# applied-ai-lab/genesis

Measured on AMD Instinct MI355X. Metric: training images/sec (fwd+bwd+GECO step), GENESIS-V2 K=7 64x64, higher is better.
Workload: dtype f32

## Files before the change

### genesis_amd/csrc/gx_norm.hip

```cpp
#include "gx_common.h"

#include <vector>

namespace {

struct View {
    float* ptr;
    int ctot;
    int c0;
    int mode;
    const float* proj;
    int projC;
    const float* pgate;
    int nsplit;
    size_t sstride;
};

struct InSrc {
    const float* p;
    int nsplit;
    size_t stride;
    const float* bias;
    float* ysum;
};
// ... 454 lines not shown
            store_view4(d0, n, c, r, col, H, W, o);
            if (d1.ptr) store_view4(d1, n, c, r, col, H, W, o);
            am = fmaxf(fmaxf(am, fmaxf(o[0], o[1])), fmaxf(o[2], o[3]));
        }
    }
    if (amax_parts) {
#pragma unroll
        for (int of = 32; of >= 1; of >>= 1) am = fmaxf(am, __shfl_xor(am, of, 64));
        if (lane == 0) amr[wave] = am;
        __syncthreads();
        if (threadIdx.x == 0) {
            float r = 0.f;
            for (int i = 0; i < (int)(blockDim.x >> 6); ++i) r = fmaxf(r, amr[i]);
            amax_parts[blockIdx.x] = r;
        }
    }
}

__device__ __forceinline__ f32x4 staged_grad(const float* gsl, const float (&pw)[8], int ctot, int HW, int i4) {
    f32x4 g = {0.f, 0.f, 0.f, 0.f};
#pragma unroll
    for (int q = 0; q < 8; ++q)
        if (q < ctot) g += pw[q] * reinterpret_cast<const f32x4*>(gsl)[q * (HW >> 2) + i4];
    return g;
}

template <int F, int UPW, bool STAGE>
__global__ void __launch_bounds__(1024)
gn_relu_bwd_reg_kernel(const float* __restrict__ y, const float* __restrict__ gamma, const float* __restrict__ beta,
                       const float* __restrict__ mean_in, const float* __restrict__ rstd_in,
// ... 485 lines not shown
    if (HW >= 256 || (W % 4) != 0 || cpg > 64 || m > 4096) return 0;
    return gx_round_up(m / 4, 64);
}

inline float* gn_take_link_out(const float* tensor, int ctot, int c0, int mode, int C, unsigned nwg, size_t covered, bool second_copy = false) {
    GxAmaxLink& L = gx_amax_link();
    const bool link_ok = !second_copy && L.parts && !L.tensor && tensor && c0 == 0 && mode == 0 && ctot == C && covered == L.numel;
    return gx_amax_producer_out(tensor, link_ok, nwg, covered);
}
template <int F, int UPW>
void launch_fwd_reg(dim3 grid, dim3 block, hipStream_t s, const InSrc src, const float* gamma, const float* beta, int C, int H,
                    int W, int groups, int P, float eps, View d0, View d1, float* mean, float* rstd) {
    float* ap = d0.ptr ? gn_take_link_out(d0.ptr, d0.ctot, d0.c0, d0.mode, C, grid.x, (size_t)(grid.x / groups) * C * H * W, d1.ptr != nullptr) : nullptr;
    hipLaunchKernelGGL((gn_relu_fwd_reg_kernel<F, UPW>), grid, block, 0, s, src, gamma, beta, C, H, W, groups, P, eps, d0, d1,
                       mean, rstd, ap);
}
template <int F, int UPW>
bool launch_bwd_stage(dim3 grid, dim3 block, hipStream_t s, size_t lds, const float* y, const float* gamma,
                      const float* beta, const float* mean, const float* rstd, int C, int H, int W, int groups, int P,
                      View g0, View g1, float* dy, float* part, float* wpart, float* bpart) {
    if (UPW != 1 || block.x != 1024 || g0.ctot != 4) return false;
    float* amax_parts = gn_take_link_out(dy, C, 0, 0, C, grid.x, (size_t)(grid.x / groups) * C * H * W);
    constexpr bool KEEP = F < 8;
    static bool attr_set = false;
    if (!attr_set) {
        (void)hipFuncSetAttribute(reinterpret_cast<const void*>(&gn_relu_bwd_stage_kernel<F, 4, true, KEEP>),
                                  hipFuncAttributeMaxDynamicSharedMemorySize, 150 * 1024);
        (void)hipFuncSetAttribute(reinterpret_cast<const void*>(&gn_relu_bwd_stage_kernel<F, 4, false, KEEP>),
                                  hipFuncAttributeMaxDynamicSharedMemorySize, 150 * 1024);
        attr_set = true;
// ... 374 lines not shown
                               beta, C, H, W, groups, pl.P, eps, d0, d1, mean, rstd);
        else if (st)
            hipLaunchKernelGGL(gn_relu_fwd_small_kernel, dim3(N * groups), dim3(st), 0, (hipStream_t)stream, src, gamma,
                               beta, C, H, W, groups, eps, d0, d1, mean, rstd);
        else {
            float* ap = dst0 ? gn_take_link_out(dst0, d0.ctot, d0.c0, d0.mode, C, (unsigned)(N * groups), (size_t)N * C * H * W, dst1 != nullptr) : nullptr;
            if (vec)
                hipLaunchKernelGGL(gn_relu_fwd_kernel<true>, dim3(N * groups), dim3(threads), 0, (hipStream_t)stream, src,
                                   gamma, beta, C, H, W, groups, eps, d0, d1, mean, rstd, ap);
            else
                hipLaunchKernelGGL(gn_relu_fwd_kernel<false>, dim3(N * groups), dim3(threads), 0, (hipStream_t)stream, src,
                                   gamma, beta, C, H, W, groups, eps, d0, d1, mean, rstd, ap);
        }
    }
    GX_CHECK_LAUNCH("gx_gn_relu_fwd");
    return GX_OK;
}

size_t gx_gn_relu_bwd_ws_bytes(int N, int C) { return (size_t)N * C * 3 * sizeof(float); }
size_t gx_gn_relu_bwd_proj_ws_bytes(int N, int C, int H, int W, int groups, int Cout) {
    size_t b = gx_gn_relu_bwd_ws_bytes(N, C);
    if (proj_split_ok(C, H, W, groups, Cout))
        b += ((size_t)N * groups * (H * W / kSplitPix) * kSplitRec + (size_t)N * groups * 2) * sizeof(float);
    return b;
}

static int gn_relu_bwd_impl(const float* y, const float* gamma, const float* beta, const float* mean,
                            const float* rstd, int N, int C, int H, int W, int groups, const View& v0, const View& v1,
                            float* dy, float* dgamma, float* dbeta, float* dbias, void* ws, size_t ws_bytes,
                            gx_stream_t stream, float* wpart = nullptr, float* bpart = nullptr);
// ... 140 lines not shown
```

### genesis_amd/csrc/gx_slots.hip

```cpp
#include "gx_common.h"

#include <cstdlib>

namespace {

constexpr int KMAX = 16;

__device__ __forceinline__ float block_sum_f(float v, float* red) {
    v = gx_wave_sum(v);
    const int lane = threadIdx.x & 63, wave = threadIdx.x >> 6, nw = blockDim.x >> 6;
    __syncthreads();
    if (lane == 0) red[wave] = v;
    __syncthreads();
    float s = 0.f;
    for (int i = 0; i < nw; ++i) s += red[i];
    return s;
}
__device__ __forceinline__ double block_sum_dd(double v, double* red) {
    v = gx_wave_sum_d(v);
    const int lane = threadIdx.x & 63, wave = threadIdx.x >> 6, nw = blockDim.x >> 6;
    __syncthreads();
    if (lane == 0) red[wave] = v;
    __syncthreads();
    double s = 0.0;
// ... 126 lines not shown
#pragma unroll
        for (int k = 0; k < KMAX; ++k) {
            if (k < K) {
                const float g = gsh[k * C + c];
                a[k] += g * fv;
                d += m[k] * g;
            }
        }
        dfb[(size_t)c * HW] = d;
    }
#pragma unroll
    for (int k = 0; k < KMAX; ++k)
        if (k < K) dlog_m[k * kstride + (size_t)b * HW + p] = m[k] * (a[k] + gmsum[(size_t)b * K + k]);
}

template <int KT>
__global__ void __launch_bounds__(256)
maskpool_bwd_vec_kernel(const float* __restrict__ f, const float* __restrict__ log_m, const float* __restrict__ gS,
                        const float* __restrict__ gmsum, int B, int C, int HW, int Krt, float* __restrict__ df,
                        float* __restrict__ dlog_m) {
    const int K = KT ? KT : Krt;
    constexpr int KMAX = KT ? KT : ::KMAX;
    extern __shared__ __attribute__((aligned(16))) float sm[];
    float* gsh = sm;
    f32x4* ared = reinterpret_cast<f32x4*>(sm + ((K * C + 3) & ~3));
    const int lane = threadIdx.x & 63, wave = threadIdx.x >> 6;
    const int b = blockIdx.x;
    const int p = (blockIdx.y * 64 + lane) * 4;
    for (int i = threadIdx.x; i < K * C; i += blockDim.x) gsh[i] = gS[(size_t)b * K * C + i];
    __syncthreads();
    const bool act = p < HW;
    const size_t kstride = (size_t)B * HW;
    f32x4 m[KMAX], a[KMAX];
#pragma unroll
    for (int k = 0; k < KMAX; ++k) {
        a[k][0] = 0.f; a[k][1] = 0.f; a[k][2] = 0.f; a[k][3] = 0.f;
        m[k] = a[k];
        if (k < K && act) {
            const f32x4 lm = *reinterpret_cast<const f32x4*>(log_m + k * kstride + (size_t)b * HW + p);
#pragma unroll
            for (int e = 0; e < 4; ++e) m[k][e] = expf(lm[e]);
        }
    }
    const int cper = (C + 3) / 4;
    const int cbeg = wave * cper, cend = (cbeg + cper < C) ? cbeg + cper : C;
    if (act) {
        const float* fb = f + (size_t)b * C * HW + p;
        float* dfb = df + (size_t)b * C * HW + p;
#pragma unroll 4
        for (int c = cbeg; c < cend; ++c) {
            const f32x4 fv = *reinterpret_cast<const f32x4*>(fb + (size_t)c * HW);
            f32x4 d = {0.f, 0.f, 0.f, 0.f};
#pragma unroll
            for (int k = 0; k < KMAX; ++k) {
                if (k < K) {
                    const float g = gsh[k * C + c];
                    a[k] += g * fv;
                    d += m[k] * g;
                }
            }
            *reinterpret_cast<f32x4*>(dfb + (size_t)c * HW) = d;
        }
    }
#pragma unroll
    for (int k = 0; k < KMAX; ++k)
        if (k < K) ared[(wave * K + k) * 64 + lane] = a[k];
    __syncthreads();
    if (wave == 0 && act) {
#pragma unroll
        for (int k = 0; k < KMAX; ++k) {
            if (k < K) {
                const f32x4 t = (ared[(0 * K + k) * 64 + lane] + ared[(1 * K + k) * 64 + lane]) +
                                (ared[(2 * K + k) * 64 + lane] + ared[(3 * K + k) * 64 + lane]);
                *reinterpret_cast<f32x4*>(dlog_m + k * kstride + (size_t)b * HW + p) =
                    m[k] * (t + gmsum[(size_t)b * K + k]);
            }
        }
    }
}

constexpr float LOG_SQRT_2PI = 0.91893853320467274178f;

template <bool BWD, int KT>
__global__ void __launch_bounds__(256)
mixture_kernel(const float* __restrict__ x, const float* __restrict__ dec, int B, int HW, int Krt, float std_,
               int pixel_bound, float* __restrict__ recon, float* __restrict__ x_r, float* __restrict__ log_m_r,
               float* __restrict__ err_part, const float* __restrict__ g_err, float* __restrict__ ddec,
               const float* __restrict__ log_w, float* __restrict__ dlog_w, float std_first, int DC) {
    const int K = KT ? KT : Krt;
    constexpr int KMAX = KT ? KT : ::KMAX;
// ... 450 lines not shown
#undef GX_MP_FWD
    }
    GX_CHECK_LAUNCH("gx_maskpool_fwd");
    return GX_OK;
}

int gx_maskpool_bwd(const float* f, const float* log_m, const float* gS, const float* gmsum, int B, int C, int H,
                    int W, int K, float* df, float* dlog_m, gx_stream_t stream) {
    GX_CHECK_ARG(f && log_m && gS && gmsum && df && dlog_m, "gx_maskpool_bwd: null pointer");
    GX_CHECK_ARG(B > 0 && C > 0 && K >= 1 && K <= KMAX && H > 0 && W > 0, "gx_maskpool_bwd: bad dims (K<=16)");
    const int HW = H * W;
    {
        GxProf pf(KID_MASKPOOL_BWD, (hipStream_t)stream, 4.0 * B * K * C * HW, 4.0 * B * HW * (2.0 * C + 2.0 * K));
        if (gx_vec4_ok(HW, f, log_m, df, dlog_m)) {
#define GX_MP_BWD(KT_)                                                                                                 \
            hipLaunchKernelGGL(maskpool_bwd_vec_kernel<KT_>, dim3(B, gx_ceil_div(HW, 256)), dim3(256),                \
                               (size_t)(((K * C + 3) & ~3) + 4 * K * 64 * 4) * sizeof(float), (hipStream_t)stream, f,   \
                               log_m, gS, gmsum, B, C, HW, K, df, dlog_m)
            if (K == 7) GX_MP_BWD(7); else if (K == 5) GX_MP_BWD(5); else if (K == 11) GX_MP_BWD(11); else GX_MP_BWD(0);
#undef GX_MP_BWD
        }
        else
            hipLaunchKernelGGL(maskpool_bwd_kernel, dim3(B, gx_ceil_div(HW, 256)), dim3(256),
                               (size_t)K * C * sizeof(float), (hipStream_t)stream, f, log_m, gS, gmsum, B, C, HW, K, df,
                               dlog_m);
    }
    GX_CHECK_LAUNCH("gx_maskpool_bwd");
    return GX_OK;
}

size_t gx_mixture_ws_bytes(int B, int H, int W) { return (size_t)B * gx_ceil_div(H * W, 256) * sizeof(float); }

static int mixture_fwd_impl(const float* x, const float* dec, const float* log_w, int dec_ch, int B, int H, int W, int K,
                            float std_first, float pixel_std, int pixel_bound, float* recon, float* x_r,
                            float* log_m_r, float* err, void* ws, size_t ws_bytes, gx_stream_t stream) {
    GX_CHECK_ARG(x && dec && recon && x_r && err && ws, "gx_mixture_fwd: null pointer");
    GX_CHECK_ARG(B > 0 && K >= 1 && K <= KMAX && pixel_std > 0.f, "gx_mixture_fwd: bad dims (K<=16)");
    GX_CHECK_ARG(ws_bytes >= gx_mixture_ws_bytes(B, H, W), "gx_mixture_fwd: workspace too small");
    const int HW = H * W, nb = gx_ceil_div(HW, 256);
    hipStream_t s = (hipStream_t)stream;
    {
        GxProf pf(KID_MIXTURE_FWD, s, 0.0, 4.0 * B * HW * (6.0 + 8.0 * K));
// ... 297 lines not shown
```

### genesis_amd/functions.py

```python
import os

import torch
import torch.nn.functional as F

from . import _lib
from . import autostep as _auto
from . import hip_ops as hip
from . import precision as _precision

GROUPS = 8
EPS = 1e-5

class _StepState(object):
    __slots__ = ('direct_param_grads', 'direct_written', 'async_wgrad', 'side_stream', 'keep_alive', 'early_flush')

    def __init__(self):
        self.direct_param_grads = False
        self.direct_written = set()
        self.async_wgrad = False
        self.side_stream = None
        self.keep_alive = []
        self.early_flush = None


# ... 385 lines not shown
    @staticmethod
    def forward(ctx, enc_feat, seg_w, seg_gamma, seg_beta, conv_w, conv_b, gate, uv, log_sigma, rand_pixel, K, kernel,
                seed_idx, min_mass, feat_w, feat_gamma, feat_beta):
        x = enc_feat.contiguous()
        ctx.am_x = getattr(enc_feat, '_gx_amax', None)
        ctx.params = (seg_w, seg_gamma, seg_beta, conv_w, conv_b, gate, log_sigma, feat_w, feat_gamma, feat_beta)
        w2 = conv_w.detach().view(conv_w.shape[0], -1)
        y, yf, ctx.pair_ws = hip.conv3x3_pair_fwd(x, seg_w, feat_w, amax_in=ctx.am_x)
        mean, rstd = hip.gn_relu_fwd(y, seg_gamma, seg_beta, GROUPS, EPS, None)
        colour = hip.conv1x1_gn_fwd(y, mean, rstd, seg_gamma, seg_beta, GROUPS, w2, conv_b, gate, uv)
        ctx.ls_dtype = log_sigma.dtype
        ls64 = log_sigma.detach().to(torch.float64)
        res = hip.icsbp_fwd(colour, ls64, rand_pixel.contiguous(), K, kernel, seed_idx, min_mass)
        log_m, log_s, seeds, idx = res[:4]
        ctx.nsteps = res[4] if min_mass > 0.0 else None
        f = torch.empty_like(yf)
        meanf, rstdf = hip.gn_relu_fwd(yf, feat_gamma, feat_beta, GROUPS, EPS, (f, 0, 0))
        ctx.save_for_backward(x, y, mean, rstd, ls64, colour, seeds, idx, yf, meanf, rstdf)
        ctx.kernel = kernel
        ctx.mark_non_differentiable(idx)
        ctx.set_materialize_grads(False)
        if ctx.nsteps is not None:
            ctx.mark_non_differentiable(ctx.nsteps)
            return log_m, log_s, colour, seeds, idx, ctx.nsteps, f
        return log_m, log_s, colour, seeds, idx, f

    @staticmethod
    def backward(ctx, g_log_m, *rest):
        _refuse_grads('SegFeatHeadsFn', rest)
        x, y, mean, rstd, ls64, colour, seeds, idx, yf, meanf, rstdf = ctx.saved_tensors
        seg_w, seg_gamma, seg_beta, conv_w, conv_b, gate, log_sigma, feat_w, feat_gamma, feat_beta = ctx.params
        g_f = rest[-1]
        if g_log_m is None:
            g_log_m = colour.new_zeros(seeds.shape[0] + 1, colour.shape[0], 1, colour.shape[2], colour.shape[3])
        if g_f is None:
            g_f = torch.zeros_like(yf)
        ols = _gout(log_sigma) if ctx.ls_dtype == torch.float64 and log_sigma.dim() == 0 else None
        dcolour, dls = hip.icsbp_bwd(colour, ls64, seeds, idx, g_log_m.contiguous(), ctx.kernel, out_dls=ols,
                                     nsteps=ctx.nsteps)
        w2 = conv_w.detach().view(conv_w.shape[0], -1)
        ow, ob, og = _gout(conv_w), _gout(conv_b), (_gout(gate) if gate is not None else None)
        osw, osg, osb = _gout(seg_w), _gout(seg_gamma), _gout(seg_beta)
        fused = hip.conv1x1_gn_bwd_fused(y, seg_gamma, seg_beta, mean, rstd, GROUPS, dcolour, w2, conv_b, gate, False,
                                         out_gn=(osg, osb, None), out_conv=(ow, ob, og))
        if fused is not None:
            dy, (dgamma, dbeta, _), (dw, db, dgate) = fused
        else:
            dw, db, dgate = hip.conv1x1_gn_wgrad(y, mean, rstd, seg_gamma, seg_beta, GROUPS, dcolour, w2, conv_b, gate,
                                                 out=(ow, ob, og))
            dy, dgamma, dbeta, _ = hip.gn_relu_bwd_proj(y, seg_gamma, seg_beta, mean, rstd, GROUPS, dcolour, w2, False,
                                                        out=(osg, osb, None), gate=gate)
        am_s = (hip.take_amax(), ctx.am_x)
        dsw = _wgrad(lambda: hip.conv3x3_wgrad(x, dy, out=osw, amax=am_s), osw, x, dy)
        ofw, ofg, ofb = _gout(feat_w), _gout(feat_gamma), _gout(feat_beta)
        dyf, dfgamma, dfbeta, _ = hip.gn_relu_bwd(yf, feat_gamma, feat_beta, meanf, rstdf, GROUPS, (g_f.contiguous(), 0, 0),
                                                  out=(ofg, ofb, None))
        am_f = (hip.take_amax(), ctx.am_x)
        dfw = _wgrad(lambda: hip.conv3x3_wgrad(x, dyf, out=ofw, amax=am_f), ofw, x, dyf)
        dx = hip.conv3x3_pair_dgrad(dy, dyf, seg_w, feat_w, ctx.pair_ws, amax_in=[am_s[0], am_f[0]]) if ctx.needs_input_grad[0] else None
        return (dx, _ret(osw, dsw), _ret(osg, dgamma), _ret(osb, dbeta), _ret(ow, dw.view(conv_w.shape)), _ret(ob, db),
                _ret(og, dgate), None, _ret(ols, dls.to(ctx.ls_dtype)), None, None, None, None, None,
                _ret(ofw, dfw), _ret(ofg, dfgamma), _ret(ofb, dfbeta))


@ctx_bound
class MaskPoolFn(torch.autograd.Function):
    @staticmethod
    def forward(ctx, f, log_m):
        f = f.contiguous()
        log_m = log_m.contiguous()
        S, msum = hip.maskpool_fwd(f, log_m)
        ctx.save_for_backward(f, log_m)
        return S, msum

    @staticmethod
    def backward(ctx, gS, gmsum):
        f, log_m = ctx.saved_tensors
# ... 933 lines not shown
```

### genesis_amd/genesisv2_config.py

```python
import math

import numpy as np
import torch
import torch.nn as nn
import torch.nn.functional as F
from torch.distributions.normal import Normal

from genesis_amd import autostep
from genesis_amd import compat as _compat

_compat.install()

from attrdict import AttrDict
from forge import flags

from genesis_amd import functions as fn
from genesis_amd.lazy import Lazy, LazyAttrDict, SlotList
from genesis_amd import hip_ops as hip

flags.DEFINE_integer('feat_dim', 64, 'Number of features and latents.')
flags.DEFINE_string('kernel', 'gaussian', '{laplacian, gaussian, epanechnikov')
flags.DEFINE_boolean('semiconv', True, 'Use semi-convolutional embeddings.')
flags.DEFINE_boolean('dynamic_K', False, 'Dynamic K.')
flags.DEFINE_boolean('klm_loss', False, 'KL mask regulariser.')
# ... 209 lines not shown
        K, D = self.K_steps, self.feat_dim
        dev = x.device
        uv, _ = self._grid(dev)
        enc_feat = fn.UNetEncoderFn.apply(x, self.encoder.num_blocks, 8, *self.encoder.flat_params())
        if rand_pixel is None and eps is None and getattr(self, 'noise', None) is not None:
            rand_pixel, eps = self.noise((B, 1, H, W), (K, B, D), dev)
        if rand_pixel is None:
            rand_pixel = torch.rand(B, 1, H, W, device=dev)
        ap = self.att_process
        if ap.semiconv:
            cw, cb, gate, addend = ap.colour_head.conv.weight, ap.colour_head.conv.bias, ap.colour_head.gate.gate, uv
        else:
            cw, cb, gate, addend = ap.colour_head.weight, ap.colour_head.bias, None, None
        seg_params = self.seg_head.params()
        min_mass = 20.0 if self.dynamic_K else 0.0
        f = None
        if fn.heads_pairable(enc_feat, seg_params[0], cw, self.feat_head[0].params()[0]):
            res = fn.SegFeatHeadsFn.apply(enc_feat, *seg_params, cw, cb, gate, addend, ap.log_sigma, rand_pixel, K,
                                          ap.kernel, seed_idx, min_mass, *self.feat_head[0].params())
            res, f = res[:-1], res[-1]
        elif fn.seg_head_fusable(enc_feat, seg_params[0], cw):
            res = fn.SegICSBPFn.apply(enc_feat, *seg_params, cw, cb, gate, addend, ap.log_sigma, rand_pixel, K, ap.kernel,
                                      seed_idx, min_mass)
        else:
            seg = fn.ConvGNReLUFn.apply(enc_feat, *seg_params)
            res = fn.ICSBPFn.apply(seg, cw, cb, gate, addend, ap.log_sigma, rand_pixel, K, ap.kernel, seed_idx, min_mass)
        log_m, log_s, colour, seeds, idx = res[:5]
        dyn_batched = False
        if self.dynamic_K:
            if B == 1:
                n = int(res[5][0])
                K = n + 1
                log_m, log_s = log_m[:K], log_s[:K]
                seeds, idx = seeds[:min(n + 1, self.K_steps - 1)], idx[:min(n + 1, self.K_steps - 1)]
                if eps is not None:
                    eps = eps[:K]
            else:
                dyn_batched = True
        if f is None:
            f = fn.ConvGNReLUFn.apply(enc_feat, *self.feat_head[0].params())
        S, msum = fn.MaskPoolFn.apply(f, log_m)
        ln = self.z_head[0]
        zh = fn.PooledHeadFn.apply(fn.linear(S, self.feat_head[1].weight), msum, self.feat_head[1].bias,
                                   ln.weight, ln.bias, ln.eps)
        if eps is None:
            eps = torch.randn(K, B, D, device=dev)
        zh = fn.linear(zh, self.z_head[1].weight, self.z_head[1].bias, 'relu')
        zh = fn.linear(zh, self.z_head[3].weight, self.z_head[3].bias)
        z, mu, sigma, log_q = fn.PosteriorFn.apply(zh, eps)
        err, recon, x_r, log_m_r = self._decode(z, x, self.klm_loss and not self.detach_mr_in_klm)
        kl = self._component_kl(z, log_q)
        t = dict(err=err, kl=kl, recon=recon, log_m=log_m, log_s=log_s, x_r=x_r, log_m_r=log_m_r, colour=colour, seeds=seeds,
                 idx=idx, mu=mu, sigma=sigma, z=z)
        if self.klm_loss:
            t['kl_m'] = fn.CategoricalKLFn.apply(log_m, log_m_r.detach() if self.detach_mr_in_klm else log_m_r)
        t['dyn_batched'] = dyn_batched
# ... 75 lines not shown
```

### genesis_amd/hip_ops.py

```python
import ctypes
import os

import torch

from . import _lib
from ._lib import GenesisHipError

F32 = torch.float32
KERNELS = {'gaussian': 0, 'laplacian': 1, 'epanechnikov': 2}


def _chk(t, name, dtype=F32):
    if t is None:
        return
    if not t.is_cuda:
        raise GenesisHipError('%s: the HIP hot path needs device tensors (got %s); there is no CPU fallback'
                              % (name, t.device))
    if t.dtype != dtype:
        raise GenesisHipError('%s: expected %s, got %s' % (name, dtype, t.dtype))
    if not t.is_contiguous():
        raise GenesisHipError('%s: tensor must be contiguous' % name)


def _p(t):
# ... 542 lines not shown
    msum = torch.empty(B, K, dtype=F32, device=f.device)
    _lib.call('gx_maskpool_fwd', _p(f), _p(log_m), B, C, H, W, K, _p(S), _p(msum), _stream())
    return S, msum


def maskpool_bwd(f, log_m, gS, gmsum):
    _chk(gS, 'maskpool_bwd.gS'); _chk(gmsum, 'maskpool_bwd.gmsum')
    B, C, H, W = f.shape
    K = log_m.shape[0]
    df = torch.empty_like(f)
    dlog_m = torch.empty_like(log_m)
    _lib.call('gx_maskpool_bwd', _p(f), _p(log_m), _p(gS), _p(gmsum), B, C, H, W, K, _p(df), _p(dlog_m), _stream())
    return df, dlog_m


def mixture_fwd(x, dec, K, pixel_std, pixel_bound=True):
    _chk(x, 'mixture.x'); _chk(dec, 'mixture.dec')
    B, _, H, W = x.shape
    assert dec.shape == (K * B, 4, H, W), dec.shape
    dev = x.device
    recon = torch.empty(B, 3, H, W, dtype=F32, device=dev)
    x_r = torch.empty(K, B, 3, H, W, dtype=F32, device=dev)
    log_m_r = torch.empty(K, B, 1, H, W, dtype=F32, device=dev)
    err = torch.empty(B, dtype=F32, device=dev)
    nb = _lib.query('gx_mixture_ws_bytes', B, H, W)
    ws = _ws(nb, dev)
    _lib.call('gx_mixture_fwd', _p(x), _p(dec), B, H, W, K, float(pixel_std), int(bool(pixel_bound)), _p(recon),
              _p(x_r), _p(log_m_r), _p(err), _p(ws), nb, _stream())
    return err, recon, x_r, log_m_r

# ... 867 lines not shown
```

### include/genesis_hip.h

```cpp
#ifndef GENESIS_HIP_H
#define GENESIS_HIP_H
#include <stddef.h>
#include <stdint.h>

#ifdef __cplusplus
extern "C" {
#endif

typedef void* gx_stream_t;

#define GX_OK 0
#define GX_EINVAL (-1)
#define GX_ELAUNCH (-2)
#define GX_EDATA (-3)

const char* gx_last_error(void);
int gx_version(void);

size_t gx_conv3x3_ws_bytes(int N, int Cin, int Cout, int H, int W);
int gx_conv3x3_fwd(const float* x, const float* w, float* y, int N, int Cin, int Cout, int H, int W,
                   void* ws, size_t ws_bytes, gx_stream_t stream);
int gx_conv3x3_dgrad(const float* dy, const float* w, float* dx, int N, int Cin, int Cout, int H, int W,
                     void* ws, size_t ws_bytes, gx_stream_t stream);
int gx_conv3x3_dgrad_parts(const float* dy, const float* w, float* dx, int N, int Cin, int Cout, int H, int W, void* ws,
// ... 40 lines not shown
int gx_deconv5x5s2_fwd(const float* x, const float* w, const float* bias, float* y, int N, int Cin, int Cout,
                       int Hin, int Win, void* ws, size_t ws_bytes, gx_stream_t stream);
size_t gx_deconv5x5s2_gn_stats_ws_bytes(int N, int Cin, int Cout, int Hin, int Win);
int gx_deconv5x5s2_gn_stats_fwd(const float* x, const float* w, const float* bias, float* y, int N, int Cin, int Cout,
                                int Hin, int Win, int groups, float eps, float* mean, float* rstd, int* fused,
                                void* ws, size_t ws_bytes, gx_stream_t stream);
int gx_deconv5x5s2_dgrad(const float* dy, const float* w, float* dx, int N, int Cin, int Cin_out, int Cout,
                         int Hin, int Win, void* ws, size_t ws_bytes, gx_stream_t stream);
size_t gx_deconv5x5s2_wgrad_ws_bytes(int N, int Cin, int Cout, int Hin, int Win);
int gx_deconv5x5s2_wgrad(const float* x, const float* dy, float* dw, int N, int Cin, int Cout, int Hin, int Win,
                         void* ws, size_t ws_bytes, gx_stream_t stream);

int gx_gn_relu_fwd(const float* y, const float* gamma, const float* beta, int N, int C, int H, int W, int groups,
                   float eps, float* dst0, int dst0_ctot, int dst0_c0, int dst0_mode, float* dst1, int dst1_ctot,
                   int dst1_c0, int dst1_mode, float* mean, float* rstd, gx_stream_t stream);
size_t gx_gn_relu_bwd_ws_bytes(int N, int C);
int gx_gn_relu_bwd(const float* y, const float* gamma, const float* beta, const float* mean, const float* rstd,
                   int N, int C, int H, int W, int groups, const float* g0, int g0_ctot, int g0_c0, int g0_mode,
                   const float* g1, int g1_ctot, int g1_c0, int g1_mode, float* dy, float* dgamma, float* dbeta,
                   float* dbias, void* ws, size_t ws_bytes, gx_stream_t stream);
int gx_gn_relu_bwd_parts(const float* y, const float* gamma, const float* beta, const float* mean, const float* rstd,
                         int N, int C, int H, int W, int groups, const float* g0, int g0_ctot, int g0_c0, int g0_mode,
                         int g0_nsplit, size_t g0_split_stride, const float* g1, int g1_ctot, int g1_c0, int g1_mode,
                         int g1_nsplit, size_t g1_split_stride, float* dy, float* dgamma, float* dbeta, float* dbias, void* ws,
                         size_t ws_bytes, gx_stream_t stream);
int gx_gn_relu_bwd_proj(const float* y, const float* gamma, const float* beta, const float* mean, const float* rstd,
                        int N, int C, int H, int W, int groups, const float* g_out, int Cout, const float* w,
                        const float* gate, float* dy, float* dgamma, float* dbeta, float* dbias, float* wpart,
                        float* bpart, void* ws, size_t ws_bytes, gx_stream_t stream);
int gx_gn_relu_bwd_proj_fuses_wgrad(int C, int H, int W, int groups, int Cout);
// ... 7 lines not shown
size_t gx_icsbp_bwd_ws_bytes(int B, int H, int W, int K);
int gx_icsbp_bwd(const float* colour, const double* log_sigma, const float* seeds, const int64_t* seed_idx,
                 const float* g_log_m, int B, int C, int H, int W, int K, int kernel_type, float* dcolour,
                 double* dlog_sigma, void* ws, size_t ws_bytes, gx_stream_t stream);
int gx_icsbp_fwd_dyn(const float* colour, const double* log_sigma, const float* rand_pixel, const int64_t* seed_idx_in,
                     int B, int C, int H, int W, int K, int kernel_type, float min_mass, float* log_m, float* log_s,
                     float* seeds, int64_t* seed_idx_out, int* nsteps, gx_stream_t stream);
int gx_icsbp_bwd_dyn(const float* colour, const double* log_sigma, const float* seeds, const int64_t* seed_idx,
                     const float* g_log_m, const int* nsteps, int B, int C, int H, int W, int K, int kernel_type,
                     float* dcolour, double* dlog_sigma, void* ws, size_t ws_bytes, gx_stream_t stream);

int gx_maskpool_fwd(const float* f, const float* log_m, int B, int C, int H, int W, int K, float* S, float* msum,
                    gx_stream_t stream);
int gx_maskpool_bwd(const float* f, const float* log_m, const float* gS, const float* gmsum, int B, int C, int H,
                    int W, int K, float* df, float* dlog_m, gx_stream_t stream);

size_t gx_mixture_ws_bytes(int B, int H, int W);
int gx_mixture_fwd(const float* x, const float* dec, int B, int H, int W, int K, float pixel_std, int pixel_bound,
                   float* recon, float* x_r, float* log_m_r, float* err, void* ws, size_t ws_bytes,
                   gx_stream_t stream);
int gx_mixture_bwd(const float* x, const float* dec, const float* g_err, int B, int H, int W, int K,
                   float pixel_std, int pixel_bound, float* ddec, gx_stream_t stream);

int gx_conv1x1_fwd(const float* x, const float* w, const float* bias, const float* gate, const float* addend,
                   int N, int Cin, int Cout, int H, int W, float* y, gx_stream_t stream);
size_t gx_conv1x1_bwd_ws_bytes(int N, int Cin, int Cout, int H, int W);
int gx_conv1x1_bwd(const float* x, const float* dy, const float* w, const float* bias, const float* gate, int N,
                   int Cin, int Cout, int H, int W, float* dx, float* dw, float* db, float* dgate, void* ws,
                   size_t ws_bytes, gx_stream_t stream);
int gx_conv1x1_bwd_ex(const float* x, const float* dy, const float* w, const float* bias, const float* gate, int N,
// ... 315 lines not shown
```

Baseline: 11730.

## Fuse feature GroupNorm+ReLU with mask pooling and recompute features in pool backward

```diff
diff --git a/genesis_amd/csrc/gx_norm.hip b/genesis_amd/csrc/gx_norm.hip
--- a/genesis_amd/csrc/gx_norm.hip
+++ b/genesis_amd/csrc/gx_norm.hip
@@ -492,6 +492,114 @@
             for (int i = 0; i < (int)(blockDim.x >> 6); ++i) r = fmaxf(r, amr[i]);
             amax_parts[blockIdx.x] = r;
         }
+    }
+}
+
+constexpr int kPoolKMax = 16;
+constexpr size_t kPoolLdsBudget = 128 * 1024;
+template <int F, int UPW>
+__global__ void __launch_bounds__(1024)
+gn_relu_fwd_pool_kernel(const float* __restrict__ x, const float* __restrict__ gamma, const float* __restrict__ beta,
+                        const float* __restrict__ log_m, int C, int H, int W, int groups, int P, int K, float eps,
+                        float* __restrict__ mean_out, float* __restrict__ rstd_out, float* __restrict__ S,
+                        float* __restrict__ msum) {
+    __shared__ double red[16 * 2 + 2];
+    __shared__ double upool[32][kPoolKMax];
+    extern __shared__ __attribute__((aligned(16))) float msl[];
+    const int n = blockIdx.x / groups, gidx = blockIdx.x % groups;
+    const int N = gridDim.x / groups;
+    const int cpg = C / groups, HW = H * W;
+    const int m = cpg * HW;
+    const int lane = threadIdx.x & 63, wave = threadIdx.x >> 6;
+    const int q4 = (HW >> 2) / P;
+    const size_t slab_off = ((size_t)n * C + (size_t)gidx * cpg) * HW;
+    f32x4 xr[UPW][F];
+    double acc[2] = {0.0, 0.0};
+#pragma unroll
+    for (int u = 0; u < UPW; ++u) {
+        const int unit = wave * UPW + u;
+        const int cl = unit / P, part = unit - cl * P;
+#pragma unroll
+        for (int j = 0; j < F; ++j)
+            xr[u][j] = *reinterpret_cast<const f32x4*>(x + slab_off + (size_t)cl * HW + 4 * (size_t)(part * q4 + j * 64 + lane));
+    }
+    {
+        const int HW4 = HW >> 2, lHW4 = __ffs(HW4) - 1;
+#pragma unroll 2
+        for (int i = threadIdx.x; i < K * HW4; i += blockDim.x) {
+            const int k = i >> lHW4, p4 = i & (HW4 - 1);
+            const f32x4 lm = *reinterpret_cast<const f32x4*>(log_m + ((size_t)k * N + n) * HW + 4 * (size_t)p4);
+            f32x4 mv;
+#pragma unroll
+            for (int e = 0; e < 4; ++e) mv[e] = expf(lm[e]);
+            reinterpret_cast<f32x4*>(msl)[i] = mv;
+        }
+    }
+#pragma unroll
+    for (int u = 0; u < UPW; ++u)
+#pragma unroll
+        for (int j = 0; j < F; ++j) {
+            const f32x4 v = xr[u][j];
+            acc[0] += ((double)v[0] + (double)v[1]) + ((double)v[2] + (double)v[3]);
+            acc[1] += ((double)v[0] * v[0] + (double)v[1] * v[1]) + ((double)v[2] * v[2] + (double)v[3] * v[3]);
+        }
+    block_sum_multi<2>(acc, red);
+    const double mean = acc[0] / m;
+    double var = acc[1] / m - mean * mean;
+    if (var < 0.0) var = 0.0;
+    const float meanf = (float)mean;
+    const float rstdf = (float)(1.0 / sqrt(var + (double)eps));
+    if (threadIdx.x == 0) { mean_out[blockIdx.x] = meanf; rstd_out[blockIdx.x] = rstdf; }
+#pragma unroll
+    for (int u = 0; u < UPW; ++u) {
+        const int unit = wave * UPW + u;
+        const int cl = unit / P;
+        const int c = gidx * cpg + cl;
+        const float gm = gamma[c], bt = beta[c];
+#pragma unroll
+        for (int j = 0; j < F; ++j)
+#pragma unroll
+            for (int e = 0; e < 4; ++e) {
+                const float t = (xr[u][j][e] - meanf) * rstdf * gm + bt;
+                xr[u][j][e] = t > 0.f ? t : 0.f;
+            }
+    }
+    const f32x4* ms4 = reinterpret_cast<const f32x4*>(msl);
+    for (int k = 0; k < K; ++k) {
+#pragma unroll
+        for (int u = 0; u < UPW; ++u) {
+            const int unit = wave * UPW + u;
+            const int cl = unit / P, part = unit - cl * P;
+            double s0 = 0.0, s1 = 0.0, s2 = 0.0, s3 = 0.0;
+#pragma unroll
+            for (int j = 0; j < F; ++j) {
+                const f32x4 mv = ms4[k * (HW >> 2) + part * q4 + j * 64 + lane];
+                s0 += (double)(mv[0] * xr[u][j][0]);
+                s1 += (double)(mv[1] * xr[u][j][1]);
+                s2 += (double)(mv[2] * xr[u][j][2]);
+                s3 += (double)(mv[3] * xr[u][j][3]);
+            }
+            const double s = gx_wave_sum_d((s0 + s1) + (s2 + s3));
+            if (lane == 0) upool[unit][k] = s;
+        }
+    }
+    if (gidx == 0) {
+        for (int k = wave; k < K; k += (int)(blockDim.x >> 6)) {
+            double s0 = 0.0, s1 = 0.0, s2 = 0.0, s3 = 0.0;
+            for (int i = lane; i < (HW >> 2); i += 64) {
+                const f32x4 mv = ms4[k * (HW >> 2) + i];
+                s0 += (double)mv[0]; s1 += (double)mv[1]; s2 += (double)mv[2]; s3 += (double)mv[3];
+            }
+            const double s = gx_wave_sum_d((s0 + s1) + (s2 + s3));
+            if (lane == 0) msum[(size_t)n * K + k] = (float)s;
+        }
+    }
+    __syncthreads();
+    for (int t = threadIdx.x; t < cpg * K; t += blockDim.x) {
+        const int cl = t / K, k = t - cl * K;
+        double s = 0.0;
+        for (int p = 0; p < P; ++p) s += upool[cl * P + p][k];
+        S[((size_t)n * K + k) * C + gidx * cpg + cl] = (float)s;
     }
 }
 
@@ -1007,6 +1115,19 @@
     float* ap = d0.ptr ? gn_take_link_out(d0.ptr, d0.ctot, d0.c0, d0.mode, C, grid.x, (size_t)(grid.x / groups) * C * H * W, d1.ptr != nullptr) : nullptr;
     hipLaunchKernelGGL((gn_relu_fwd_reg_kernel<F, UPW>), grid, block, 0, s, src, gamma, beta, C, H, W, groups, P, eps, d0, d1,
                        mean, rstd, ap);
+}
+template <int F, int UPW>
+void launch_fwd_pool(dim3 grid, dim3 block, hipStream_t s, size_t lds, const float* y, const float* gamma, const float* beta,
+                     const float* log_m, int C, int H, int W, int groups, int P, int K, float eps, float* mean, float* rstd,
+                     float* S, float* msum) {
+    static bool attr_set = false;
+    if (!attr_set) {
+        (void)hipFuncSetAttribute(reinterpret_cast<const void*>(&gn_relu_fwd_pool_kernel<F, UPW>),
+                                  hipFuncAttributeMaxDynamicSharedMemorySize, (int)kPoolLdsBudget);
+        attr_set = true;
+    }
+    hipLaunchKernelGGL((gn_relu_fwd_pool_kernel<F, UPW>), grid, block, lds, s, y, gamma, beta, log_m, C, H, W, groups, P, K, eps,
+                       mean, rstd, S, msum);
 }
 template <int F, int UPW>
 bool launch_bwd_stage(dim3 grid, dim3 block, hipStream_t s, size_t lds, const float* y, const float* gamma,
@@ -1411,6 +1532,37 @@
         }
     }
     GX_CHECK_LAUNCH("gx_gn_relu_fwd");
+    return GX_OK;
+}
+
+int gx_gn_relu_pool_covers(const float* y, const float* log_m, size_t lm_stride_k, size_t lm_stride_n, size_t lm_stride_h,
+                           size_t lm_stride_w, int N, int C, int H, int W, int groups, int K) {
+    if (N <= 0 || C <= 0 || groups <= 0 || C % groups || K < 1 || K > kPoolKMax) return 0;
+    if (H < 2 || W < 2 || !gx_is_pow2(H) || !gx_is_pow2(W)) return 0;
+    if (!plan_reg(C / groups, H, W).ok) return 0;
+    if ((size_t)K * H * W * sizeof(float) > kPoolLdsBudget) return 0;
+    if (gx_maskpool_bwd_norm_lds_bytes(C, K) > 64 * 1024) return 0;
+    if (lm_stride_w != 1 || lm_stride_h != (size_t)W || lm_stride_n != (size_t)H * W || lm_stride_k != (size_t)N * H * W) return 0;
+    if (((reinterpret_cast<uintptr_t>(y) | reinterpret_cast<uintptr_t>(log_m)) & 15) != 0) return 0;
+    return 1;
+}
+
+int gx_gn_relu_pool_fwd(const float* y, const float* gamma, const float* beta, const float* log_m, size_t lm_stride_k,
+                        size_t lm_stride_n, size_t lm_stride_h, size_t lm_stride_w, int N, int C, int H, int W, int groups,
+                        int K, float eps, float* mean, float* rstd, float* S, float* msum, int* covered,
+                        gx_stream_t stream) {
+    GX_CHECK_ARG(y && gamma && beta && log_m && mean && rstd && S && msum && covered, "gx_gn_relu_pool_fwd: null pointer");
+    *covered = gx_gn_relu_pool_covers(y, log_m, lm_stride_k, lm_stride_n, lm_stride_h, lm_stride_w, N, C, H, W, groups, K);
+    if (!*covered) return GX_OK;
+    {
+        const double el = (double)N * C * H * W;
+        GxProf pf(KID_GN_FWD, (hipStream_t)stream, 8.0 * el + 2.0 * K * el, 4.0 * el + 4.0 * (double)N * K * H * W);
+        const RegPlan pl = plan_reg(C / groups, H, W);
+        GX_GN_REG_DISPATCH(launch_fwd_pool, pl, dim3(N * groups), dim3(pl.threads), (hipStream_t)stream,
+                           (size_t)K * H * W * sizeof(float), y, gamma, beta, log_m, C, H, W, groups, pl.P, K, eps, mean, rstd,
+                           S, msum);
+    }
+    GX_CHECK_LAUNCH("gx_gn_relu_pool_fwd");
     return GX_OK;
 }
 
diff --git a/genesis_amd/csrc/gx_slots.hip b/genesis_amd/csrc/gx_slots.hip
--- a/genesis_amd/csrc/gx_slots.hip
+++ b/genesis_amd/csrc/gx_slots.hip
@@ -164,11 +164,24 @@
         if (k < K) dlog_m[k * kstride + (size_t)b * HW + p] = m[k] * (a[k] + gmsum[(size_t)b * K + k]);
 }
 
-template <int KT>
+__device__ __forceinline__ f32x4 add_rounded_product(f32x4 g, f32x4 m, f32x4 v) {
+#pragma clang fp contract(off)
+    const f32x4 r = m * v;
+    return g + r;
+}
+struct PoolNorm {
+    const float* mean;
+    const float* rstd;
+    const float* gamma;
+    const float* beta;
+    int groups;
+    const float* g_add;
+};
+template <int KT, bool NORM>
 __global__ void __launch_bounds__(256)
 maskpool_bwd_vec_kernel(const float* __restrict__ f, const float* __restrict__ log_m, const float* __restrict__ gS,
                         const float* __restrict__ gmsum, int B, int C, int HW, int Krt, float* __restrict__ df,
-                        float* __restrict__ dlog_m) {
+                        float* __restrict__ dlog_m, const PoolNorm nrm) {
     const int K = KT ? KT : Krt;
     constexpr int KMAX = KT ? KT : ::KMAX;
     extern __shared__ __attribute__((aligned(16))) float sm[];
@@ -178,6 +191,16 @@
     const int b = blockIdx.x;
     const int p = (blockIdx.y * 64 + lane) * 4;
     for (int i = threadIdx.x; i < K * C; i += blockDim.x) gsh[i] = gS[(size_t)b * K * C + i];
+    f32x4* nsh = reinterpret_cast<f32x4*>(sm + ((K * C + 3) & ~3) + 4 * K * 64 * 4);
+    if (NORM) {
+        const int cpg = C / nrm.groups;
+        for (int c = threadIdx.x; c < C; c += blockDim.x) {
+            const int sl = b * nrm.groups + c / cpg;
+            f32x4 t;
+            t[0] = nrm.mean[sl]; t[1] = nrm.rstd[sl]; t[2] = nrm.gamma[c]; t[3] = nrm.beta[c];
+            nsh[c] = t;
+        }
+    }
     __syncthreads();
     const bool act = p < HW;
     const size_t kstride = (size_t)B * HW;
@@ -199,7 +222,16 @@
         float* dfb = df + (size_t)b * C * HW + p;
 #pragma unroll 4
         for (int c = cbeg; c < cend; ++c) {
-            const f32x4 fv = *reinterpret_cast<const f32x4*>(fb + (size_t)c * HW);
+            f32x4 fv = *reinterpret_cast<const f32x4*>(fb + (size_t)c * HW);
+            if (NORM) {
+                const f32x4 nc = nsh[c];
+                const float meanf = nc[0], rstdf = nc[1], gm = nc[2], bt = nc[3];
+#pragma unroll
+                for (int e = 0; e < 4; ++e) {
+                    const float t = (fv[e] - meanf) * rstdf * gm + bt;
+                    fv[e] = t > 0.f ? t : 0.f;
+                }
+            }
             f32x4 d = {0.f, 0.f, 0.f, 0.f};
 #pragma unroll
             for (int k = 0; k < KMAX; ++k) {
@@ -222,8 +254,12 @@
             if (k < K) {
                 const f32x4 t = (ared[(0 * K + k) * 64 + lane] + ared[(1 * K + k) * 64 + lane]) +
                                 (ared[(2 * K + k) * 64 + lane] + ared[(3 * K + k) * 64 + lane]);
-                *reinterpret_cast<f32x4*>(dlog_m + k * kstride + (size_t)b * HW + p) =
-                    m[k] * (t + gmsum[(size_t)b * K + k]);
+                const f32x4 v = t + gmsum[(size_t)b * K + k];
+                f32x4* out = reinterpret_cast<f32x4*>(dlog_m + k * kstride + (size_t)b * HW + p);
+                if (NORM && nrm.g_add)
+                    *out = add_rounded_product(*reinterpret_cast<const f32x4*>(nrm.g_add + k * kstride + (size_t)b * HW + p), m[k], v);
+                else
+                    *out = m[k] * v;
             }
         }
     }
@@ -704,9 +740,9 @@
         GxProf pf(KID_MASKPOOL_BWD, (hipStream_t)stream, 4.0 * B * K * C * HW, 4.0 * B * HW * (2.0 * C + 2.0 * K));
         if (gx_vec4_ok(HW, f, log_m, df, dlog_m)) {
 #define GX_MP_BWD(KT_)                                                                                                 \
-            hipLaunchKernelGGL(maskpool_bwd_vec_kernel<KT_>, dim3(B, gx_ceil_div(HW, 256)), dim3(256),                \
+            hipLaunchKernelGGL((maskpool_bwd_vec_kernel<KT_, false>), dim3(B, gx_ceil_div(HW, 256)), dim3(256),       \
                                (size_t)(((K * C + 3) & ~3) + 4 * K * 64 * 4) * sizeof(float), (hipStream_t)stream, f,   \
-                               log_m, gS, gmsum, B, C, HW, K, df, dlog_m)
+                               log_m, gS, gmsum, B, C, HW, K, df, dlog_m, PoolNorm{})
             if (K == 7) GX_MP_BWD(7); else if (K == 5) GX_MP_BWD(5); else if (K == 11) GX_MP_BWD(11); else GX_MP_BWD(0);
 #undef GX_MP_BWD
         }
@@ -716,6 +752,34 @@
                                dlog_m);
     }
     GX_CHECK_LAUNCH("gx_maskpool_bwd");
+    return GX_OK;
+}
+
+size_t gx_maskpool_bwd_norm_lds_bytes(int C, int K) {
+    return (size_t)(((K * C + 3) & ~3) + 4 * K * 64 * 4 + 4 * C) * sizeof(float);
+}
+
+int gx_maskpool_bwd_norm(const float* y, const float* mean, const float* rstd, const float* gamma, const float* beta,
+                         int groups, const float* log_m, const float* gS, const float* gmsum, const float* g_log_m, int B,
+                         int C, int H, int W, int K, float* df, float* dlog_m, gx_stream_t stream) {
+    GX_CHECK_ARG(y && mean && rstd && gamma && beta && log_m && gS && gmsum && df && dlog_m, "gx_maskpool_bwd_norm: null pointer");
+    GX_CHECK_ARG(B > 0 && C > 0 && K >= 1 && K <= KMAX && H > 0 && W > 0, "gx_maskpool_bwd_norm: bad dims (K<=16)");
+    GX_CHECK_ARG(groups > 0 && C % groups == 0, "gx_maskpool_bwd_norm: C must be a multiple of groups");
+    GX_CHECK_ARG(gx_maskpool_bwd_norm_lds_bytes(C, K) <= 64 * 1024, "gx_maskpool_bwd_norm: K * (C + 1024) + C floats of LDS exceed 64 KB");
+    const int HW = H * W;
+    GX_CHECK_ARG(gx_vec4_ok(HW, y, log_m, df, dlog_m) && gx_vec4_ok(HW, g_log_m),
+                 "gx_maskpool_bwd_norm: H*W %% 4 == 0 and 16-byte aligned tensors");
+    {
+        GxProf pf(KID_MASKPOOL_BWD, (hipStream_t)stream, 4.0 * B * K * C * HW, 4.0 * B * HW * (2.0 * C + (g_log_m ? 3.0 : 2.0) * K));
+        const PoolNorm nrm{mean, rstd, gamma, beta, groups, g_log_m};
+#define GX_MP_BWD(KT_)                                                                                                 \
+        hipLaunchKernelGGL((maskpool_bwd_vec_kernel<KT_, true>), dim3(B, gx_ceil_div(HW, 256)), dim3(256),            \
+                           gx_maskpool_bwd_norm_lds_bytes(C, K), (hipStream_t)stream, y,                               \
+                           log_m, gS, gmsum, B, C, HW, K, df, dlog_m, nrm)
+        if (K == 7) GX_MP_BWD(7); else if (K == 5) GX_MP_BWD(5); else if (K == 11) GX_MP_BWD(11); else GX_MP_BWD(0);
+#undef GX_MP_BWD
+    }
+    GX_CHECK_LAUNCH("gx_maskpool_bwd_norm");
     return GX_OK;
 }
 
diff --git a/genesis_amd/functions.py b/genesis_amd/functions.py
--- a/genesis_amd/functions.py
+++ b/genesis_amd/functions.py
@@ -423,23 +423,41 @@
         res = hip.icsbp_fwd(colour, ls64, rand_pixel.contiguous(), K, kernel, seed_idx, min_mass)
         log_m, log_s, seeds, idx = res[:4]
         ctx.nsteps = res[4] if min_mass > 0.0 else None
-        f = torch.empty_like(yf)
-        meanf, rstdf = hip.gn_relu_fwd(yf, feat_gamma, feat_beta, GROUPS, EPS, (f, 0, 0))
-        ctx.save_for_backward(x, y, mean, rstd, ls64, colour, seeds, idx, yf, meanf, rstdf)
+        ctx.pooled = hip.FEAT_POOL_FUSE and hip.gn_relu_pool_covers(yf, log_m, GROUPS)
+        if ctx.pooled:
+            meanf, rstdf, S, msum, _ = hip.gn_relu_pool_fwd(yf, feat_gamma, feat_beta, GROUPS, EPS, log_m)
+            tail = (S, msum)
+        else:
+            f = torch.empty_like(yf)
+            meanf, rstdf = hip.gn_relu_fwd(yf, feat_gamma, feat_beta, GROUPS, EPS, (f, 0, 0))
+            tail = (f,)
+        ctx.save_for_backward(x, y, mean, rstd, ls64, colour, seeds, idx, yf, meanf, rstdf, log_m)
         ctx.kernel = kernel
         ctx.mark_non_differentiable(idx)
         ctx.set_materialize_grads(False)
         if ctx.nsteps is not None:
             ctx.mark_non_differentiable(ctx.nsteps)
-            return log_m, log_s, colour, seeds, idx, ctx.nsteps, f
-        return log_m, log_s, colour, seeds, idx, f
+            return (log_m, log_s, colour, seeds, idx, ctx.nsteps) + tail
+        return (log_m, log_s, colour, seeds, idx) + tail
 
     @staticmethod
     def backward(ctx, g_log_m, *rest):
+        x, y, mean, rstd, ls64, colour, seeds, idx, yf, meanf, rstdf, log_m = ctx.saved_tensors
+        seg_w, seg_gamma, seg_beta, conv_w, conv_b, gate, log_sigma, feat_w, feat_gamma, feat_beta = ctx.params
+        if ctx.pooled:
+            gS, gmsum = rest[-2], rest[-1]
+            rest = rest[:-2]
+            if gS is None and gmsum is None:
+                g_f = None
+            else:
+                gS = gS.contiguous() if gS is not None else yf.new_zeros(yf.shape[0], log_m.shape[0], yf.shape[1])
+                gmsum = gmsum.contiguous() if gmsum is not None else yf.new_zeros(yf.shape[0], log_m.shape[0])
+                g_f, g_log_m = hip.maskpool_bwd_norm(yf, meanf, rstdf, feat_gamma, feat_beta, GROUPS, log_m, gS, gmsum,
+                                                     g_log_m.contiguous() if g_log_m is not None else None)
+        else:
+            g_f = rest[-1]
+            rest = rest[:-1]
         _refuse_grads('SegFeatHeadsFn', rest)
-        x, y, mean, rstd, ls64, colour, seeds, idx, yf, meanf, rstdf = ctx.saved_tensors
-        seg_w, seg_gamma, seg_beta, conv_w, conv_b, gate, log_sigma, feat_w, feat_gamma, feat_beta = ctx.params
-        g_f = rest[-1]
         if g_log_m is None:
             g_log_m = colour.new_zeros(seeds.shape[0] + 1, colour.shape[0], 1, colour.shape[2], colour.shape[3])
         if g_f is None:
@@ -470,6 +488,12 @@
         return (dx, _ret(osw, dsw), _ret(osg, dgamma), _ret(osb, dbeta), _ret(ow, dw.view(conv_w.shape)), _ret(ob, db),
                 _ret(og, dgate), None, _ret(ols, dls.to(ctx.ls_dtype)), None, None, None, None, None,
                 _ret(ofw, dfw), _ret(ofg, dfgamma), _ret(ofb, dfbeta))
+
+
+def split_heads(res):
+    if res[-1].dim() == 2:
+        return res[:-2], None, res[-2], res[-1]
+    return res[:-1], res[-1], None, None
 
 
 @ctx_bound
diff --git a/genesis_amd/genesisv2_config.py b/genesis_amd/genesisv2_config.py
--- a/genesis_amd/genesisv2_config.py
+++ b/genesis_amd/genesisv2_config.py
@@ -247,11 +247,11 @@
             cw, cb, gate, addend = ap.colour_head.weight, ap.colour_head.bias, None, None
         seg_params = self.seg_head.params()
         min_mass = 20.0 if self.dynamic_K else 0.0
-        f = None
+        f = S = msum = None
         if fn.heads_pairable(enc_feat, seg_params[0], cw, self.feat_head[0].params()[0]):
             res = fn.SegFeatHeadsFn.apply(enc_feat, *seg_params, cw, cb, gate, addend, ap.log_sigma, rand_pixel, K,
                                           ap.kernel, seed_idx, min_mass, *self.feat_head[0].params())
-            res, f = res[:-1], res[-1]
+            res, f, S, msum = fn.split_heads(res)
         elif fn.seg_head_fusable(enc_feat, seg_params[0], cw):
             res = fn.SegICSBPFn.apply(enc_feat, *seg_params, cw, cb, gate, addend, ap.log_sigma, rand_pixel, K, ap.kernel,
                                       seed_idx, min_mass)
@@ -270,9 +270,13 @@
                     eps = eps[:K]
             else:
                 dyn_batched = True
-        if f is None:
-            f = fn.ConvGNReLUFn.apply(enc_feat, *self.feat_head[0].params())
-        S, msum = fn.MaskPoolFn.apply(f, log_m)
+        if S is not None:
+            if K < S.shape[1]:
+                S, msum = S[:, :K], msum[:, :K]
+        else:
+            if f is None:
+                f = fn.ConvGNReLUFn.apply(enc_feat, *self.feat_head[0].params())
+            S, msum = fn.MaskPoolFn.apply(f, log_m)
         ln = self.z_head[0]
         zh = fn.PooledHeadFn.apply(fn.linear(S, self.feat_head[1].weight), msum, self.feat_head[1].bias,
                                    ln.weight, ln.bias, ln.eps)
diff --git a/genesis_amd/hip_ops.py b/genesis_amd/hip_ops.py
--- a/genesis_amd/hip_ops.py
+++ b/genesis_amd/hip_ops.py
@@ -580,6 +580,64 @@
     return df, dlog_m
 
 
+FEAT_POOL_FUSE = os.environ.get('GENESIS_FEAT_POOL_FUSE', '1') != '0'
+
+
+def _lm_strides(log_m):
+    assert log_m.dim() == 5 and log_m.shape[2] == 1, log_m.shape
+    s = log_m.stride()
+    return [ctypes.c_size_t(max(int(v), 0)) for v in (s[0], s[1], s[3], s[4])]
+
+
+def gn_relu_pool_covers(y, log_m, groups):
+    N, C, H, W = y.shape
+    if not (y.is_cuda and log_m.is_cuda and y.dtype == F32 and log_m.dtype == F32 and y.is_contiguous()):
+        return False
+    if log_m.dim() != 5 or log_m.shape[1:] != (N, 1, H, W) or min(log_m.stride()) < 0:
+        return False
+    return bool(_lib.load().gx_gn_relu_pool_covers(_p(y), _p(log_m), *_lm_strides(log_m), N, C, H, W, groups, log_m.shape[0]))
+
+
+def gn_relu_pool_fwd(y, gamma, beta, groups, eps, log_m, fuse=None):
+    _chk(y, 'gn_pool.y'); _chk(gamma, 'gn_pool.gamma'); _chk(beta, 'gn_pool.beta')
+    if not log_m.is_cuda or log_m.dtype != F32:
+        _chk(log_m, 'gn_pool.log_m')
+    N, C, H, W = y.shape
+    K = log_m.shape[0]
+    assert log_m.shape == (K, N, 1, H, W), (log_m.shape, y.shape)
+    if (FEAT_POOL_FUSE if fuse is None else fuse) and min(log_m.stride()) >= 0:
+        mean = torch.empty(N * groups, dtype=F32, device=y.device)
+        rstd = torch.empty(N * groups, dtype=F32, device=y.device)
+        S = torch.empty(N, K, C, dtype=F32, device=y.device)
+        msum = torch.empty(N, K, dtype=F32, device=y.device)
+        covered = ctypes.c_int(0)
+        _lib.call('gx_gn_relu_pool_fwd', _p(y), _p(gamma), _p(beta), _p(log_m), *_lm_strides(log_m), N, C, H, W, groups, K,
+                  float(eps), _p(mean), _p(rstd), _p(S), _p(msum), ctypes.byref(covered), _stream())
+        if covered.value:
+            _probe_gn(y, gamma, beta, mean, rstd, groups)
+            return mean, rstd, S, msum, None
+    f = torch.empty_like(y)
+    mean, rstd = gn_relu_fwd(y, gamma, beta, groups, eps, (f, 0, 0))
+    S, msum = maskpool_fwd(f, log_m.contiguous())
+    return mean, rstd, S, msum, f
+
+
+def maskpool_bwd_norm(y, mean, rstd, gamma, beta, groups, log_m, gS, gmsum, g_log_m=None):
+    _chk(y, 'maskpool_bwd_norm.y'); _chk(mean, 'maskpool_bwd_norm.mean'); _chk(rstd, 'maskpool_bwd_norm.rstd')
+    _chk(gamma, 'maskpool_bwd_norm.gamma'); _chk(beta, 'maskpool_bwd_norm.beta'); _chk(log_m, 'maskpool_bwd_norm.log_m')
+    _chk(gS, 'maskpool_bwd_norm.gS'); _chk(gmsum, 'maskpool_bwd_norm.gmsum'); _chk(g_log_m, 'maskpool_bwd_norm.g_log_m')
+    B, C, H, W = y.shape
+    K = log_m.shape[0]
+    assert log_m.shape == (K, B, 1, H, W) and gS.shape == (B, K, C) and gmsum.shape == (B, K), (log_m.shape, gS.shape, gmsum.shape)
+    assert mean.numel() == B * groups and rstd.numel() == B * groups and gamma.numel() == C and beta.numel() == C
+    assert g_log_m is None or g_log_m.shape == log_m.shape, g_log_m.shape
+    df = torch.empty_like(y)
+    dlog_m = torch.empty_like(log_m)
+    _lib.call('gx_maskpool_bwd_norm', _p(y), _p(mean), _p(rstd), _p(gamma), _p(beta), groups, _p(log_m), _p(gS), _p(gmsum),
+              _p(g_log_m), B, C, H, W, K, _p(df), _p(dlog_m), _stream())
+    return df, dlog_m
+
+
 def mixture_fwd(x, dec, K, pixel_std, pixel_bound=True):
     _chk(x, 'mixture.x'); _chk(dec, 'mixture.dec')
     B, _, H, W = x.shape
diff --git a/include/genesis_hip.h b/include/genesis_hip.h
--- a/include/genesis_hip.h
+++ b/include/genesis_hip.h
@@ -78,6 +78,12 @@
 int gx_gn_relu_fwd(const float* y, const float* gamma, const float* beta, int N, int C, int H, int W, int groups,
                    float eps, float* dst0, int dst0_ctot, int dst0_c0, int dst0_mode, float* dst1, int dst1_ctot,
                    int dst1_c0, int dst1_mode, float* mean, float* rstd, gx_stream_t stream);
+int gx_gn_relu_pool_covers(const float* y, const float* log_m, size_t lm_stride_k, size_t lm_stride_n, size_t lm_stride_h,
+                           size_t lm_stride_w, int N, int C, int H, int W, int groups, int K);
+int gx_gn_relu_pool_fwd(const float* y, const float* gamma, const float* beta, const float* log_m, size_t lm_stride_k,
+                        size_t lm_stride_n, size_t lm_stride_h, size_t lm_stride_w, int N, int C, int H, int W, int groups,
+                        int K, float eps, float* mean, float* rstd, float* S, float* msum, int* covered,
+                        gx_stream_t stream);
 size_t gx_gn_relu_bwd_ws_bytes(int N, int C);
 int gx_gn_relu_bwd(const float* y, const float* gamma, const float* beta, const float* mean, const float* rstd,
                    int N, int C, int H, int W, int groups, const float* g0, int g0_ctot, int g0_c0, int g0_mode,
@@ -115,6 +121,10 @@
                     gx_stream_t stream);
 int gx_maskpool_bwd(const float* f, const float* log_m, const float* gS, const float* gmsum, int B, int C, int H,
                     int W, int K, float* df, float* dlog_m, gx_stream_t stream);
+size_t gx_maskpool_bwd_norm_lds_bytes(int C, int K);
+int gx_maskpool_bwd_norm(const float* y, const float* mean, const float* rstd, const float* gamma, const float* beta,
+                         int groups, const float* log_m, const float* gS, const float* gmsum, const float* g_log_m, int B,
+                         int C, int H, int W, int K, float* df, float* dlog_m, gx_stream_t stream);
 
 size_t gx_mixture_ws_bytes(int B, int H, int W);
 int gx_mixture_fwd(const float* x, const float* dec, int B, int H, int W, int K, float pixel_std, int pixel_bound,
```

Result: no change. 11810 (median of 6 runs) (+0.7%).
